# anenbergb/Co-DETR-TensorRT

Measured on AMD Instinct MI355X. Metric: images/sec, Co-DINO Swin-L 1920x1280 fp16 (p50 ms/image alongside), higher is better.
Workload: dtype f16

## Files before the change

### __graft_entry__.py

```python
import os
import subprocess
import sys

ROOT = os.path.dirname(os.path.abspath(__file__))
PKG_ROOT = os.path.join(ROOT, "co-detr-tensorrt_amd")
for _p in (ROOT, PKG_ROOT, os.path.join(ROOT, "oracle")):
    if _p not in sys.path:
        sys.path.insert(0, _p)


def _newer(target, sources):
    if not os.path.isfile(target):
        return True
    t = os.path.getmtime(target)
    return any(os.path.getmtime(s) > t for s in sources)


def build() -> None:
    csrc = os.path.join(PKG_ROOT, "csrc")
    so = os.path.join(PKG_ROOT, "codetr", "libcodetr_hip.so")
    srcs = [os.path.join(csrc, f) for f in os.listdir(csrc) if f.endswith((".hip", ".h", "Makefile"))]
    srcs += [os.path.join(ROOT, "include", h) for h in ("codetr_hip.h", "codetr_jpeg.h", "codetr_assign.h")]
    if _newer(so, srcs):
        subprocess.check_call(["make", "-C", csrc, "-s", "-j4"])
    runner_dir = os.path.join(ROOT, "runner")
    runner = os.path.join(runner_dir, "codetr_runner")
    if _newer(runner, [os.path.join(runner_dir, f) for f in ("codetr_runner.cpp", "dispatch_gen.inc", "Makefile")]):
        subprocess.check_call(["make", "-C", runner_dir, "-s"])
    import msda_oracle

    msda_oracle.build()
    import codetr


def smoke() -> None:
    build()
    import smoke_impl

    smoke_impl.run()


if __name__ == "__main__":
    build()
    print("build ok")
    if len(sys.argv) > 1 and sys.argv[1] == "smoke":
        smoke()
        print("smoke ok")
```

### co-detr-tensorrt_amd/codetr/_kernel_names.py

```python
KERNEL_NAMES = (
    "add_kernel",
    "assign_kernel",
    "batched_nms_kernel",
    "cast_fp8_kernel",
    "cast_fp8mx_kernel",
    "conv_im2col_nchw_kernel",
    "conv_tokens_kernel",
    "decode_boxes_kernel",
    "decoder_layer_kernel",
    "draw_detections_kernel",
    "encoder_geometry_kernel",
    "ffn_fp8_kernel",
    "ffn_fused_kernel",
    "frames_to_rgb_kernel",
    "gather_rows_kernel",
    "gn_apply_kernel",
    "gn_finalize_kernel",
    "gn_partial_kernel",
    "im2col_tokens_kernel",
    "jpeg_encode_rows_kernel",
    "jpeg_gather_rows_kernel",
    "layernorm_fp8_kernel",
    "layernorm_fp8mx_kernel",
    "layernorm_kernel",
    "level_cums_kernel",
    "level_mask_kernel",
    "linear_256_fp8_kernel",
    "linear_256_kernel",
    "linear_kernel",
    "linear_pp_kernel",
    "linear_sk_kernel",
    "linear_xs_kernel",
    "maxpool_tokens_kernel",
    "mha_attention_kernel",
    "msda_backward_generic_kernel",
    "msda_backward_kernel",
    "msda_encoder_v4_kernel",
    "msda_fused_headmajor_kernel",
    "msda_op4_kernel",
    "msda_scalar_kernel",
    "msda_tiled_kernel",
    "pack_w2_kernel",
    "patch_im2col_k4_kernel",
    "postprocess_kernel",
    "postprocess_softnms_kernel",
    "preprocess_batch_kernel",
    "preprocess_kernel",
    "preprocess_tiles_kernel",
    "preprocess_views_kernel",
    "query_sine_embed_kernel",
    "row_max_kernel",
    "sigmoid_kernel",
    "sine_pos_kernel",
    "slice_merge_kernel",
    "splitk_reduce_kernel",
    "swin_mlp_kernel",
    "topk_kernel",
    "topk_reg_kernel",
    "track_update2_kernel",
    "track_update_kernel",
    "tta_merge_kernel",
    "valid_ratios_kernel",
    "window_attention_kernel",
# ... 2 lines not shown
```

### co-detr-tensorrt_amd/codetr/hip_ops.py

```python

import collections
import math

import numpy as np
import torch
import torch.nn.functional as F

from . import _assign, _cabi, _jpeg

NATIVE = {"msda", "linear(f16/bf16, K%64==0)", "layer_norm(f16/bf16)", "swin_window_attention(f16, head_dim 32)",
          "msda_fused(softmax + sampling locations in-kernel)", "groupnorm_tokens(f16, 8 ch/group)",
          "sine_pos_tokens(f16, + level_embed)", "ffn_fused(f16, 256 -> hidden -> 256, ReLU, + identity)",
          "mask_pyramid(level masks + running valid counts + valid ratios)",
          "query_sine_embed(f16: sigmoid x valid ratios + sine embedding of the decoder reference boxes)",
          "encoder_geometry(f16: reference points, proposals, keep/drop state)", "row_max(f16)",
          "preprocess_image(u8 -> f16/f32, cv2-exact resize + pad + normalise + mask)", "batched_nms(f32)",
          "preprocess_batch(u8 -> f16/bf16/f32, <= 32 images of any size per launch, stacked + padded)",
          "postprocess_detections(f16/bf16/f32: threshold + sort + per-class NMS + rescale, one workgroup per image)",
          "postprocess_detections_soft(f16/bf16/f32: threshold + per-class soft-NMS (linear / naive) + max_per_img + rescale)",
          "patch_merge_layernorm(f16: Swin 2x2 gather + LayerNorm)",
          "msda_encoder_packed(f16/bf16: LDS-staged gather for the encoder's self-attention, csrc/msda_encoder4.hip)",
          "patch_embed(f16/bf16: 4x4 patch gather + GEMM)",
          "mha_attention(f16/bf16: dense softmax attention, head_dim 32, <= 1024 keys)",
          "topk(f16/bf16 rows, k <= 1024: radix select + bitonic sort)",
          "im2col_tokens(16-bit token-major maps)",
          "resnet50(f16/bf16: implicit-GEMM conv_tokens, stem window gather + GEMM, maxpool_tokens, BN folded)",
          "small_ops(f16: add, sigmoid, gather_rows, decode_boxes, valid_ratios)",
          "linear_fp8(e4m3 x e4m3, K%128==0) + layer_norm_fp8 + cast_fp8", "ffn_fp8(fused FFN, both products e4m3)"}


LINEAR_PROFILE = None
KERNEL_PROFILE = None


def _timed(name, meta, launch, device):
    if KERNEL_PROFILE is None:
        return launch()
    st = torch.cuda.current_stream(device)
    e0, e1 = torch.cuda.Event(enable_timing=True), torch.cuda.Event(enable_timing=True)
    e0.record(st)
    r = launch()
# ... 69 lines not shown
                    launch = lambda: _cabi.linear_splitk(x2, w, bias, r2, act, out, splits, ws, mk)
                elif (LINEAR_PP and _persistent_ok(mk, head_major, out, x2, w, r2, bias)
                      and _cabi.linear_pp_preferred(x2.shape[0], N, K, act, r2 is not None)):
                    launch = lambda: _cabi.linear_pp(x2, w, bias, r2, act, out)
                elif (_persistent_ok(mk, head_major, out, x2, w, r2, bias)
                      and _cabi.linear_sk_preferred(x2.shape[0], N, K, act, r2 is not None)):
                    launch = lambda: _cabi.linear_sk(x2, w, bias, r2, act, out)
                else:
                    launch = lambda: _cabi.linear(x2, w, bias, r2, act, out, mk, hm_rows, hm_hd)
                _timed_linear(launch, x.device, x2.shape[0], N, K)
        if head_major:
            return out.view(x.shape[0], N // hm_hd, hm_rows, hm_hd)
        return out.view(*x.shape[:-1], N)
    if head_major:
        raise RuntimeError("head_major output exists only on the native linear (f16/bf16, K % 64 == 0)")
    y = F.linear(x, weight, bias)
    if act == "relu_res":
        if row_mask is not None:
            y = y.masked_fill(row_mask[..., None], 0.0)
        return F.relu(y + residual if residual is not None else y)
    if act == "relu":
        y = F.relu(y, inplace=True)
    elif act == "gelu":
        y = F.gelu(y)
    elif act is not None:
        raise ValueError(act)
    if row_mask is not None:
        y = y.masked_fill(row_mask[..., None], 0.0)
    if residual is not None:
        y = y + residual
    return y


LN_GEMM = True


def linear_ln_supported(x, norm_weight, weight):
    return (LN_GEMM and x.is_cuda and norm_weight is not None and norm_weight.dtype == x.dtype and weight.dtype == x.dtype
            and not torch.is_grad_enabled() and norm_weight.shape[0] == x.shape[-1]
            and _cabi.linear_xadd_supported(x.numel() // max(x.shape[-1], 1), weight.shape[0], x.shape[-1], x.dtype))


def linear_ln(x, norm_weight, norm_bias, eps, weight, bias=None, act=None):
    _gpu(x, "linear_ln")
    if linear_ln_supported(x, norm_weight, weight):
        K, N = x.shape[-1], weight.shape[0]
        x2 = x.reshape(-1, K)
        x2 = x2 if x2.is_contiguous() else x2.contiguous()
        w = weight if weight.is_contiguous() else weight.contiguous()
        out = torch.empty((x2.shape[0], N), dtype=x.dtype, device=x.device)
        with torch.cuda.device(x.device):
            ok = _timed_linear(lambda: _cabi.linear_ln(x2, norm_weight, norm_bias, eps, w, bias, act, out),
                               x.device, x2.shape[0], N, K)
        if ok:
            return out.view(*x.shape[:-1], N)
    return linear(layer_norm(x, norm_weight, norm_bias, eps), weight, bias, act=act)


XADD = True
XADD_MIN_ROWS = 0


def linear_xadd_supported(x, x_add, weight):
    return (XADD and x.is_cuda and x_add is not None and x_add.shape == x.shape and x_add.dtype == x.dtype
            and weight.dtype == x.dtype and not torch.is_grad_enabled()
            and x.numel() // max(x.shape[-1], 1) >= XADD_MIN_ROWS
# ... 1472 lines not shown
```

### co-detr-tensorrt_amd/codetr/transformer.py

```python
import math

import torch
import torch.nn as nn

from . import hip_ops
from .multi_scale_deformable_attention import MultiScaleDeformableAttention
from .transformer_layers import BaseTransformerLayer, DetrTransformerDecoderLayer, build_norm


DEC_FUSED = True
DEC_VPROJ = True


class DetrTransformerEncoder(nn.Module):
    def __init__(self, post_norm_cfg=dict(type="LN"), with_cp=-1, transformerlayers=None, num_layers=None,
                 init_cfg=None):
        super().__init__()
        if not isinstance(transformerlayers, dict):
            raise AssertionError("transformerlayers must be a dict")
        layer_cfg = dict(transformerlayers)
        if layer_cfg.pop("type") != "BaseTransformerLayer":
            raise AssertionError("encoder layers must be BaseTransformerLayer")
        self.num_layers = num_layers
        self.layers = nn.ModuleList(BaseTransformerLayer(**layer_cfg) for _ in range(num_layers))
# ... 427 lines not shown
        pos_tokens = [p.flatten(2).transpose(1, 2) for p in mlvl_pos_embeds]
        return self.forward_flat(feat, shapes, mlvl_masks, pos_tokens, reg_branches, cls_branches, forced_topk_indices,
                                 capture)

    def forward_flat(self, feat, shapes, mlvl_masks, mlvl_pos_tokens, reg_branches=None, cls_branches=None,
                     forced_topk_indices=None, capture=None, lvl_pos_embed_flat=None, mask_flat=None,
                     valid_counts=None):
        if not self.as_two_stage:
            raise AssertionError("as_two_stage must be True for DINO")
        dev = feat.device
        mask = mask_flat if mask_flat is not None else torch.cat([m.flatten(1) for m in mlvl_masks], 1)
        if lvl_pos_embed_flat is not None:
            pos = lvl_pos_embed_flat
        else:
            pos = torch.cat([p + self.level_embeds[l].view(1, 1, -1) for l, p in enumerate(mlvl_pos_tokens)], 1)
        spatial_shapes, level_start_index = _shape_tensors(shapes, dev)
        if valid_counts is not None:
            valid_ratios = hip_ops.valid_ratios(valid_counts, _level_wh(shapes, feat.dtype, dev))
        else:
            valid_ratios = torch.stack([get_valid_ratio(m, dtype=feat.dtype) for m in mlvl_masks], 1)
        native_geom = feat.is_cuda and feat.dtype in (torch.float16, torch.bfloat16) and mask.dtype == torch.bool
        if native_geom:
            reference_points, ref_by_level, proposals, row_state = hip_ops.encoder_geometry(valid_ratios, mask, shapes)
            if valid_counts is not None:
                ref_by_level._codetr_valid_counts = valid_counts
        else:
            reference_points = get_reference_points([tuple(s) for s in shapes], valid_ratios, device=dev)
            ref_by_level = reference_points[:, :, None] * valid_ratios[:, None]

        memory = self.encoder.forward_bf(feat, pos, mask, reference_points=ref_by_level, spatial_shapes=spatial_shapes,
                                         level_start_index=level_start_index)
        B = memory.shape[0]
        if native_geom:
            out_mem = hip_ops.linear(memory, self.enc_output.weight, self.enc_output.bias, row_mask=row_state)
        else:
            proposals = make_encoder_output_proposals_export(reference_points, mlvl_masks)
            proposals, out_mem = apply_mask_to_proposal_and_memory(proposals, memory, mask)
            out_mem = hip_ops.linear(out_mem, self.enc_output.weight, self.enc_output.bias)
        out_mem = hip_ops.layer_norm(out_mem, self.enc_output_norm.weight, self.enc_output_norm.bias,
                                     self.enc_output_norm.eps)
        last = self.decoder.num_layers
        cls_head = cls_branches[last]
        enc_cls = hip_ops.linear(out_mem, cls_head.weight, cls_head.bias)
        if forced_topk_indices is None:
            topk = hip_ops.topk(hip_ops.row_max(enc_cls), self.two_stage_num_proposals, want_values=False)[1]
        else:
            topk = forced_topk_indices
        sel = hip_ops.gather_rows(out_mem, topk)
        topk_coords = run_mlp(reg_branches[last], sel, residual=hip_ops.gather_rows(proposals, topk))
        qw = self.query_embed.weight
        if B == 1 or not qw.is_cuda or torch.is_grad_enabled():
            query = qw[None].expand(B, -1, -1)
        else:
            query = hip_ops.derived((qw,), f"_codetr_query_b{B}", lambda: qw.detach()[None].expand(B, -1, -1).contiguous())
        if capture is not None:
            enc_coord = run_mlp(reg_branches[last], out_mem) + proposals
            capture["topk_coords_unact"] = topk_coords
            capture.update(memory=memory, enc_outputs_class=enc_cls, enc_outputs_coord_unact=enc_coord,
                           topk_indices=topk, spatial_shapes=spatial_shapes, level_start_index=level_start_index,
                           valid_ratios=valid_ratios)
        return self.decoder.forward_bf(query, memory, mask, topk_coords, valid_ratios, reg_branches,
                                       spatial_shapes=spatial_shapes, level_start_index=level_start_index)
```

### co-detr-tensorrt_amd/csrc/gemm_f16.hip

```cpp
#include <hip/hip_runtime.h>
#include <type_traits>
#include <stdint.h>
#include <stdlib.h>

#include "codetr_hip.h"
#include "device_prims.h"
#include "gemm_epilogue.h"

namespace {

constexpr int BM = 128, BN = 128;
constexpr int kThreads = 256;
constexpr int kStagingBytes = 4 * 64 * kStagePitch;

template <class F>
__host__ __device__ __forceinline__ auto dispatch_act(int act, F f) {
  switch (act) {
    case 0: return f(std::integral_constant<int, 0>{});
    case 1: return f(std::integral_constant<int, 1>{});
    case 3: return f(std::integral_constant<int, 3>{});
    default: return f(std::integral_constant<int, 2>{});
  }
}

const unsigned short* u16(const void* p) { return static_cast<const unsigned short*>(p); }
struct Operands {
  const unsigned short *x, *w, *b, *r;
  unsigned short* y;
  const unsigned char* mk;
  Operands(const void* X, const void* W, const void* bias, const void* R, void* Y, const void* mask = nullptr)
      : x(u16(X)), w(u16(W)), b(u16(bias)), r(u16(R)), y(static_cast<unsigned short*>(Y)),
        mk(static_cast<const unsigned char*>(mask)) {}
};

template <int BKT>
__device__ __forceinline__ int sw(int row) {
  return BKT == 64 ? (row >> 1) & 7 : ((row >> 2) & 3) ^ (((row >> 2) & 1) << 1);
// ... 51 lines not shown
  static constexpr int P = BKT / 16;
  const unsigned short* src[P];
  int iy[P], ix[P], chunk8[P];
  __device__ __forceinline__ void init(const unsigned short* X, const ConvGeom& g, int M, int m0, int tid) {
    constexpr int CH = BKT / 8;
#pragma unroll
    for (int q = 0; q < P; ++q) {
      const int u = q * kThreads + tid;
      const int r = u / CH, pos = u % CH;
      chunk8[q] = (pos ^ sw<BKT>(r)) * 8;
      int m = m0 + r;
      m = m < M ? m : M - 1;
      const int b = m / g.HoWo, p = m - b * g.HoWo;
      const int oy = p / g.Wo, ox = p - oy * g.Wo;
      src[q] = X + (size_t)b * g.H * g.W * g.C + chunk8[q];
      iy[q] = oy * g.stride - g.pad;
      ix[q] = ox * g.stride - g.pad;
    }
  }
  __device__ __forceinline__ void stage(const ConvGeom& g, int k0, unsigned char* lds_tile, int wave) const {
    const int tap = k0 / g.C, c0 = k0 - tap * g.C;
    const int ky = tap / g.k, kx = tap - ky * g.k;
#pragma unroll
    for (int q = 0; q < P; ++q) {
      const int y = iy[q] + ky, x = ix[q] + kx;
      const unsigned short* s = ((unsigned)y < (unsigned)g.H && (unsigned)x < (unsigned)g.W)
                                    ? src[q] + ((size_t)y * g.W + x) * g.C + c0
                                    : g_conv_zeros + chunk8[q];
      dma_piece(s, lds_tile, q, wave);
    }
  }
};

template <class T, int ACT, bool HAS_BIAS, bool HAS_RES, int BKT, int STAGES, bool SPLITK, bool CONV>
__device__ __forceinline__ void linear_body(const unsigned short* __restrict__ X, const unsigned short* __restrict__ W,
                                            const unsigned short* __restrict__ bias,
                                            const unsigned short* __restrict__ R, unsigned short* __restrict__ Y,
                                            const unsigned char* __restrict__ row_mask, int M, int N, int K,
                                            int tiles_n, int hm_rows, int hm_hd, int kps, const ConvGeom& cg) {
  constexpr int kTileBytes = 128 * BKT * 2;
  constexpr int kStageBytes = 2 * kTileBytes;
  constexpr int LPS = 2 * (BKT / 16);
  constexpr int kLdsBytes = STAGES * kStageBytes > kStagingBytes ? STAGES * kStageBytes : kStagingBytes;
  static_assert(kLdsBytes <= 64 * 1024, "pipeline does not fit 64 KiB");
  static_assert(STAGES >= 2 && STAGES <= 4, "");
  __shared__ __attribute__((aligned(16))) unsigned char lds[kLdsBytes];
  const int tid = threadIdx.x;
  const int lane = tid & 63, wave = tid >> 6;
  const int wm = wave & 1, wn = wave >> 1;

  const unsigned tile = xcd_tile(blockIdx.x, gridDim.x);
  const int tn = tile % tiles_n, tm = tile / tiles_n;
  const int m0 = tm * BM, n0 = tn * BN;

  const int ncol = 4 * (lane >> 4);
  const bool vec_n = (N & 7) == 0;
  f32x4 acc[4][4];
#pragma unroll
  for (int i = 0; i < 4; ++i) {
    f32x4 b4 = {0.f, 0.f, 0.f, 0.f};
    if (HAS_BIAS) {
      const int n = n0 + wn * 64 + i * 16 + ncol;
      if (vec_n) {
        if (n < N) {
          const s16x4 bb = *reinterpret_cast<const s16x4*>(bias + n);
#pragma unroll
          for (int r = 0; r < 4; ++r) b4[r] = T::to_f32((unsigned short)bb[r]);
        }
      } else {
#pragma unroll
        for (int r = 0; r < 4; ++r)
          if (n + r < N) b4[r] = T::to_f32(bias[n + r]);
// ... 66 lines not shown
      const int n = n0 + wn * 64 + i * 16 + ncol;
#pragma unroll
      for (int j = 0; j < 4; ++j) {
        const int m = m0 + wm * 64 + j * 16 + frow;
        if (m >= M || n >= N) continue;
        if (vec_n) {
          *reinterpret_cast<f32x4*>(part + (size_t)m * N + n) = acc[i][j];
        } else {
#pragma unroll
          for (int r = 0; r < 4; ++r)
            if (n + r < N) part[(size_t)m * N + n + r] = acc[i][j][r];
        }
      }
    }
    return;
  }

  if (vec_n) {
    constexpr int kPitch = kStagePitch;
    unsigned char* stage = lds + wave * (64 * kPitch);
#pragma unroll
    for (int i = 0; i < 4; ++i) {
#pragma unroll
      for (int j = 0; j < 4; ++j) {
        float v[4];
#pragma unroll
        for (int r = 0; r < 4; ++r) v[r] = epi_act<ACT, HAS_RES>(acc[i][j][r]);
        *reinterpret_cast<s16x4*>(stage + (j * 16 + frow) * kPitch + (i * 16 + ncol) * 2) = T::pack4(v);
      }
    }
    __builtin_amdgcn_wave_barrier();
    const int srow = lane >> 3, schunk = lane & 7;
    const int n = n0 + wn * 64 + schunk * 8;
    s16x8 rres[8];
    if (HAS_RES) {
#pragma unroll
      for (int it = 0; it < 8; ++it) {
        int m = m0 + wm * 64 + it * 8 + srow;
        m = m < M ? m : M - 1;
        const int nn = n + 8 <= N ? n : (N >= 8 ? N - 8 : 0);
        rres[it] = *reinterpret_cast<const s16x8*>(R + (size_t)m * N + nn);
      }
    }
#pragma unroll
    for (int it = 0; it < 8; ++it) {
      const int ml = it * 8 + srow;
      const int m = m0 + wm * 64 + ml;
      if (m < M && n < N) {
        s16x8 v = *reinterpret_cast<const s16x8*>(stage + ml * kPitch + schunk * 16);
        if (row_mask) {
          const unsigned char mk = row_mask[m];
          if (mk == 2) {
#pragma unroll
            for (int e = 0; e < 8; ++e)
              v[e] = (short)T::from_f32(epi_act<ACT, HAS_RES>(HAS_BIAS ? T::to_f32(bias[n + e]) : 0.f));
          } else if (mk) {
            v = s16x8{0, 0, 0, 0, 0, 0, 0, 0};
          }
        }
        size_t off = (size_t)m * N + n;
        if (hm_hd > 0) off = epi_head_major(m, n, N, hm_rows, hm_hd);
        if (HAS_RES) {
          const s16x8 rr = rres[it];
#pragma unroll
          for (int e = 0; e < 8; ++e) v[e] = (short)epi_residual<T, ACT>((unsigned short)v[e], (unsigned short)rr[e]);
        }
// ... 29 lines not shown
                                                          const unsigned short* __restrict__ W,
                                                          const unsigned short* __restrict__ bias,
                                                          const unsigned short* __restrict__ R,
                                                          unsigned short* __restrict__ Y,
                                                          const unsigned char* __restrict__ row_mask, int M, int N,
                                                          int K, int tiles_n, int hm_rows, int hm_hd, int kps) {
  linear_body<T, ACT, HAS_BIAS, HAS_RES, BKT, STAGES, SPLITK, false>(X, W, bias, R, Y, row_mask, M, N, K, tiles_n,
                                                                     hm_rows, hm_hd, kps, ConvGeom{});
}

template <class T, int ACT, bool HAS_BIAS, bool HAS_RES, int BKT, int STAGES>
__global__ __launch_bounds__(kThreads) void conv_tokens_kernel(const unsigned short* __restrict__ X,
                                                               const unsigned short* __restrict__ W,
                                                               const unsigned short* __restrict__ bias,
                                                               const unsigned short* __restrict__ R,
                                                               unsigned short* __restrict__ Y, int M, int N, int K,
                                                               int tiles_n, ConvGeom cg) {
  linear_body<T, ACT, HAS_BIAS, HAS_RES, BKT, STAGES, false, true>(X, W, bias, R, Y, nullptr, M, N, K, tiles_n, 0, 0, 0,
                                                                   cg);
}

int pipeline_cfg(int64_t K, int64_t tiles) { return (K <= 256 && tiles > 256) ? 322 : 642; }

template <class T, int ACT, int BKT, int STAGES>
int launch_cfg(hipStream_t st, const void* X, const void* W, const void* bias, const void* R, void* Y,
               const void* mask, int M, int N, int K, int hm_rows, int hm_hd) {
  const int tiles_m = (M + BM - 1) / BM, tiles_n = (N + BN - 1) / BN;
  const dim3 grid((unsigned)(tiles_m * tiles_n)), block(kThreads);
  const Operands o(X, W, bias, R, Y, mask);
  if (bias && R) hipLaunchKernelGGL((linear_kernel<T, ACT, true, true, BKT, STAGES, false>), grid, block, 0, st, o.x, o.w, o.b, o.r, o.y, o.mk, M, N, K, tiles_n, hm_rows, hm_hd, 0);
  else if (bias) hipLaunchKernelGGL((linear_kernel<T, ACT, true, false, BKT, STAGES, false>), grid, block, 0, st, o.x, o.w, o.b, o.r, o.y, o.mk, M, N, K, tiles_n, hm_rows, hm_hd, 0);
  else if (R) hipLaunchKernelGGL((linear_kernel<T, ACT, false, true, BKT, STAGES, false>), grid, block, 0, st, o.x, o.w, o.b, o.r, o.y, o.mk, M, N, K, tiles_n, hm_rows, hm_hd, 0);
  else hipLaunchKernelGGL((linear_kernel<T, ACT, false, false, BKT, STAGES, false>), grid, block, 0, st, o.x, o.w, o.b, o.r, o.y, o.mk, M, N, K, tiles_n, hm_rows, hm_hd, 0);
  const hipError_t err = hipGetLastError();
  return err == hipSuccess ? 0 : (int)err;
}

template <class T>
__global__ __launch_bounds__(256) void splitk_reduce_kernel(const float* __restrict__ part,
                                                            const unsigned short* __restrict__ bias,
                                                            const unsigned short* __restrict__ R,
                                                            const unsigned char* __restrict__ row_mask,
                                                            unsigned short* __restrict__ Y, int M, int N, int splits,
                                                            int act) {
  const int ngroups = (N + 3) / 4;
  const long idx = (long)blockIdx.x * 256 + threadIdx.x;
  if (idx >= (long)M * ngroups) return;
  const int m = (int)(idx / ngroups), n = (int)(idx % ngroups) * 4;
  const size_t off = (size_t)m * N + n;
  const bool vec = (N & 3) == 0;
  float v[4] = {0.f, 0.f, 0.f, 0.f};
  for (int z = 0; z < splits; ++z) {
    const float* p = part + (size_t)z * M * N + off;
    if (vec) {
      const f32x4 q = *reinterpret_cast<const f32x4*>(p);
#pragma unroll
      for (int r = 0; r < 4; ++r) v[r] += q[r];
    } else {
#pragma unroll
      for (int r = 0; r < 4; ++r)
        if (n + r < N) v[r] += p[r];
    }
  }
  const unsigned char mk = row_mask ? row_mask[m] : 0;
  dispatch_act(act, [&](auto a) {
#pragma unroll
// ... 27 lines not shown
    return CODETR_E_BADARG;
  if (ws_bytes < (int64_t)splits * M * N * 4) return CODETR_E_BADARG;
  const int ktiles = (int)(K / 64), kps = (ktiles + splits - 1) / splits;
  if ((int64_t)kps * (splits - 1) >= ktiles) return CODETR_E_BADARG;
  const int tiles_m = (int)((M + BM - 1) / BM), tiles_n = (int)((N + BN - 1) / BN);
  const dim3 grid((unsigned)(tiles_m * tiles_n), (unsigned)splits), block(kThreads);
  const Operands o(X, W, bias, R, Y, mask);
  hipLaunchKernelGGL((linear_kernel<T, 0, false, false, 64, 2, true>), grid, block, 0, st, o.x, o.w, nullptr, nullptr,
                     static_cast<unsigned short*>(ws), nullptr, (int)M, (int)N, (int)K, tiles_n, 0, 0, kps);
  const long groups = (long)M * ((N + 3) / 4);
  hipLaunchKernelGGL((splitk_reduce_kernel<T>), dim3((unsigned)((groups + 255) / 256)), dim3(256), 0, st,
                     static_cast<const float*>(ws), o.b, o.r, o.mk, o.y, (int)M, (int)N, splits, act);
  const hipError_t err = hipGetLastError();
  return err == hipSuccess ? 0 : (int)err;
}

template <class T, int ACT>
int launch_act(hipStream_t st, const void* X, const void* W, const void* bias, const void* R, void* Y,
               const void* mask, int M, int N, int K, int hm_rows, int hm_hd) {
  switch (pipeline_cfg(K, (int64_t)((M + BM - 1) / BM) * ((N + BN - 1) / BN))) {
    case 322: return launch_cfg<T, ACT, 32, 2>(st, X, W, bias, R, Y, mask, M, N, K, hm_rows, hm_hd);
    default: return launch_cfg<T, ACT, 64, 2>(st, X, W, bias, R, Y, mask, M, N, K, hm_rows, hm_hd);
  }
}

#ifdef CODETR_GEMM_STAMPS
__device__ unsigned long long* g_stamps = nullptr;
#endif
#ifdef CODETR_GEMM_ABL
constexpr int kGemmAbl = CODETR_GEMM_ABL;
#else
constexpr int kGemmAbl = 0;
#endif
template <class T, int ACT, bool HAS_BIAS, bool HAS_RES, bool XDEEP = false, bool SDMA = false>
__global__ __launch_bounds__(512) void linear_256_kernel(const unsigned short* __restrict__ X,
                                                         const unsigned short* __restrict__ W,
                                                         const unsigned short* __restrict__ bias,
                                                         const unsigned short* __restrict__ R,
                                                         unsigned short* __restrict__ Y,
                                                         const unsigned char* __restrict__ row_mask, int M, int N, int K,
                                                         int tiles_n) {
  constexpr int BKT = 64, NT = 512;
#ifdef CODETR_GEMM_STAMPS
  unsigned long long st0 = 0, st1 = 0, st2 = 0, rt0 = 0;
  if (threadIdx.x == 0) {
    st0 = __builtin_amdgcn_s_memtime();
    rt0 = __builtin_amdgcn_s_memrealtime();
  }
#endif
  constexpr int kTileBytes = 256 * BKT * 2;
  constexpr int kStageBytes = 2 * kTileBytes;
  __shared__ __attribute__((aligned(16))) unsigned char lds[XDEEP ? 5 * kTileBytes : 2 * kStageBytes];
  const int tid = threadIdx.x, lane = tid & 63, wave = tid >> 6;
  const int wm = wave & 1, wn = wave >> 1;
  const unsigned tile = xcd_tile(blockIdx.x, gridDim.x);
  const int tn = tile % tiles_n, tm = tile / tiles_n;
  const int m0 = tm * 256, n0 = tn * 256;
  const int frow = lane & 15, fchunk = lane >> 4, ncol = 4 * (lane >> 4);

  f32x4 acc[4][8];
#pragma unroll
  for (int i = 0; i < 4; ++i) {
    f32x4 b4 = {0.f, 0.f, 0.f, 0.f};
    if (HAS_BIAS) {
      const int n = n0 + wn * 64 + i * 16 + ncol;
      if (n < N) {
        const s16x4 bb = *reinterpret_cast<const s16x4*>(bias + n);
#pragma unroll
        for (int r = 0; r < 4; ++r) b4[r] = T::to_f32((unsigned short)bb[r]);
      }
    }
#pragma unroll
    for (int j = 0; j < 8; ++j) acc[i][j] = b4;
  }
// ... 152 lines not shown
        lds_dma16_auto(gx[q] + koff, nbufX + (q * NT + wave * 64) * 16);
      }
    }
#pragma unroll
    for (int j = 0; j < 8; ++j)
#pragma unroll
      for (int i = 0; i < 4; ++i) {
        if (!(kGemmAbl & 2)) acc[i][j] = T::mfma(a[0][i], b[0][j], acc[i][j]);
        else if (!(kGemmAbl & 4)) asm volatile("" ::"v"(a[0][i]), "v"(b[0][j]));
      }
    __builtin_amdgcn_sched_group_barrier(0x008, 2, 0);
    __builtin_amdgcn_sched_group_barrier(0x100, 12, 0);
#pragma unroll
    for (int g = 0; g < 8; ++g) {
      __builtin_amdgcn_sched_group_barrier(0x008, 3, 0);
      __builtin_amdgcn_sched_group_barrier(0x020, 1, 0);
    }
    __builtin_amdgcn_sched_group_barrier(0x008, 6, 0);
#pragma unroll
    for (int j = 0; j < 8; ++j)
#pragma unroll
      for (int i = 0; i < 4; ++i) {
        if (!(kGemmAbl & 2)) acc[i][j] = T::mfma(a[1][i], b[1][j], acc[i][j]);
        else if (!(kGemmAbl & 4)) asm volatile("" ::"v"(a[1][i]), "v"(b[1][j]));
      }
    __builtin_amdgcn_sched_group_barrier(0x008, 32, 0);
  }
  wait_vmcnt<0>();
  __builtin_amdgcn_s_barrier();
#ifdef CODETR_GEMM_STAMPS
  if (threadIdx.x == 0) st1 = __builtin_amdgcn_s_memtime();
#endif

  constexpr int kPitch = kStagePitch;
  unsigned char* stage = lds + wave * (64 * kPitch);
  const int srow = lane >> 3, schunk = lane & 7;
  const int n = n0 + wn * 64 + schunk * 8;
  unsigned char* ytile = reinterpret_cast<unsigned char*>(Y) + ((size_t)m0 * N + n0) * 2;
#pragma unroll
  for (int h = 0; h < 2; ++h) {
#pragma unroll
    for (int i = 0; i < 4; ++i)
#pragma unroll
      for (int j = 0; j < 4; ++j) {
        float v[4];
#pragma unroll
        for (int r = 0; r < 4; ++r) v[r] = epi_act<ACT, HAS_RES>(acc[i][h * 4 + j][r]);
        *reinterpret_cast<s16x4*>(stage + (j * 16 + frow) * kPitch + (i * 16 + ncol) * 2) = T::pack4(v);
      }
    __builtin_amdgcn_wave_barrier();
    s16x8 rres[8];
    if (HAS_RES) {
#pragma unroll
      for (int it = 0; it < 8; ++it) {
        int m = m0 + wm * 128 + h * 64 + it * 8 + srow;
        m = m < M ? m : M - 1;
        rres[it] = *reinterpret_cast<const s16x8*>(R + (size_t)m * N + epi_residual_col(n, N));
      }
    }
#pragma unroll
    for (int it = 0; it < 8; ++it) {
      const int ml = it * 8 + srow;
      const int m = m0 + wm * 128 + h * 64 + ml;
      if (m < M && n < N) {
        s16x8 v = *reinterpret_cast<const s16x8*>(stage + ml * kPitch + schunk * 16);
        if (row_mask) {
// ... 13 lines not shown
        }
        const unsigned loff = ((unsigned)(wm * 128 + h * 64 + ml) * (unsigned)N + (unsigned)(wn * 64 + schunk * 8)) * 2u;
        *reinterpret_cast<s16x8*>(ytile + loff) = v;
      }
    }
    __builtin_amdgcn_wave_barrier();
  }
#ifdef CODETR_GEMM_STAMPS
  if (threadIdx.x == 0 && g_stamps) {
    st2 = __builtin_amdgcn_s_memtime();
    wait_vmcnt<0>();
    const unsigned long long st3 = __builtin_amdgcn_s_memtime();
    unsigned long long* o = g_stamps + 8 * (size_t)blockIdx.x;
    o[0] = st0; o[1] = st1; o[2] = st2; o[3] = st3; o[4] = rt0; o[5] = __builtin_amdgcn_s_memrealtime();
    o[6] = wait_dma; o[7] = wait_bar;
  }
#endif
}

bool big_applicable(int64_t M, int64_t N, int64_t K, int hm_hd) {
  if (hm_hd != 0 || K < 256 || K % 64 != 0 || N % 8 != 0) return false;
  const int64_t tn = (N + 255) / 256, tm = (M + 255) / 256;
  return tm * tn >= 200 && (N * 8 >= tn * 256 * 7 || (tn == 1 && N * 4 >= 256 * 3));
}

template <class T, int ACT>
int launch_big(hipStream_t st, const void* X, const void* W, const void* bias, const void* R, void* Y, const void* mask,
               int M, int N, int K) {
  const int tiles_m = (M + 255) / 256, tiles_n = (N + 255) / 256;
  const dim3 grid((unsigned)(tiles_m * tiles_n)), block(512);
  const Operands o(X, W, bias, R, Y, mask);
  const bool sdma = tiles_n > 1;
#define CODETR_L256S(HB, HR) \
  hipLaunchKernelGGL((linear_256_kernel<T, ACT, HB, HR, true, true>), grid, block, 0, st, o.x, o.w, o.b, o.r, o.y, o.mk, M, N, K, tiles_n)
#define CODETR_L256(HB, HR) \
  hipLaunchKernelGGL((linear_256_kernel<T, ACT, HB, HR, true, false>), grid, block, 0, st, o.x, o.w, o.b, o.r, o.y, o.mk, M, N, K, tiles_n)
  if (sdma) {
    if (bias && R) CODETR_L256S(true, true);
    else if (bias) CODETR_L256S(true, false);
    else if (R) CODETR_L256S(false, true);
    else CODETR_L256S(false, false);
  } else {
    if (bias && R) CODETR_L256(true, true);
    else if (bias) CODETR_L256(true, false);
    else if (R) CODETR_L256(false, true);
    else CODETR_L256(false, false);
  }
#undef CODETR_L256
#undef CODETR_L256S
  const hipError_t err = hipGetLastError();
  return err == hipSuccess ? 0 : (int)err;
}

#ifndef CODETR_XS_ABL
#define CODETR_XS_ABL 0
#endif
#ifdef CODETR_XS_STAMPS
__device__ unsigned long long* g_xs_stamps = nullptr;
#define XS_STAMP(i) xs_t[i] = __builtin_readcyclecounter()
#else
#define XS_STAMP(i)
#endif
struct XsPosGen {
  const float* ycum[5];
  const float* xcum[5];
  const unsigned short* level_embed;
  int H[5], W[5], start[5];
  int L, S;
  float log2_temperature, scale, eps, offset;
  int normalize;
};

template <class T, int KS, int ACT, bool HAS_RES, class OT = T, bool SPLIT = false, bool POSGEN = false>
__global__ __launch_bounds__(256) void linear_xs_kernel(const unsigned short* __restrict__ X,
                                                        const unsigned short* __restrict__ X2,
                                                        const unsigned short* __restrict__ LNG,
                                                        const unsigned short* __restrict__ LNB, float ln_eps,
                                                        const unsigned short* __restrict__ W,
                                                        const unsigned short* __restrict__ bias,
                                                        const unsigned short* __restrict__ R,
                                                        unsigned short* __restrict__ Y,
                                                        const unsigned char* __restrict__ row_mask, int M, int N, int hm_rows,
// ... 582 lines not shown
                          y_dev, M, N, K, act);
}

int codetr_linear_ln_bf16(void* stream, const void* x_dev, const void* ln_gamma_dev, const void* ln_beta_dev, float ln_eps,
                          const void* w_dev, const void* bias_dev, void* y_dev, int64_t M, int64_t N, int64_t K, int act) {
  return launch_ln<BFloatT>(static_cast<hipStream_t>(stream), x_dev, ln_gamma_dev, ln_beta_dev, ln_eps, w_dev, bias_dev,
                            y_dev, M, N, K, act);
}

int codetr_linear_xadd_f16(void* stream, const void* x_dev, const void* x_add_dev, const void* w_dev,
                           const void* bias_dev, void* y_dev, int64_t M, int64_t N, int64_t K) {
  return launch_xadd<HalfT>(static_cast<hipStream_t>(stream), x_dev, x_add_dev, w_dev, bias_dev, y_dev, M, N, K);
}

int codetr_linear_xadd_bf16(void* stream, const void* x_dev, const void* x_add_dev, const void* w_dev,
                            const void* bias_dev, void* y_dev, int64_t M, int64_t N, int64_t K) {
  return launch_xadd<BFloatT>(static_cast<hipStream_t>(stream), x_dev, x_add_dev, w_dev, bias_dev, y_dev, M, N, K);
}

int codetr_linear_f16(void* stream, const void* x_dev, const void* w_dev, const void* bias_dev, const void* residual_dev,
                      const void* row_mask_dev, void* y_dev, int64_t M, int64_t N, int64_t K, int act, int64_t hm_rows,
                      int hm_head_dim) {
  return launch<HalfT>(static_cast<hipStream_t>(stream), x_dev, w_dev, bias_dev, residual_dev, y_dev, row_mask_dev, M,
                       N, K, act, hm_rows, hm_head_dim);
}

int codetr_linear_bf16(void* stream, const void* x_dev, const void* w_dev, const void* bias_dev,
                       const void* residual_dev, const void* row_mask_dev, void* y_dev, int64_t M, int64_t N,
                       int64_t K, int act, int64_t hm_rows, int hm_head_dim) {
  return launch<BFloatT>(static_cast<hipStream_t>(stream), x_dev, w_dev, bias_dev, residual_dev, y_dev, row_mask_dev,
                         M, N, K, act, hm_rows, hm_head_dim);
}

int codetr_linear_bf16_f16out(void* stream, const void* x_dev, const void* w_dev, const void* bias_dev,
                              const void* row_mask_dev, void* y_dev, int64_t M, int64_t N, int64_t K, int64_t hm_rows,
                              int hm_head_dim) {
  if (!x_dev || !w_dev || !y_dev || M <= 0 || N <= 0 || K <= 0) return CODETR_E_BADARG;
  if (M > 0x7fffffffLL || N > 0x7fffffffLL) return CODETR_E_TOO_LARGE;
  if ((reinterpret_cast<uintptr_t>(x_dev) | reinterpret_cast<uintptr_t>(w_dev) | reinterpret_cast<uintptr_t>(y_dev)) & 15) return CODETR_E_BADARG;
  if (hm_head_dim != 0 || hm_rows != 0) {
    if (hm_head_dim <= 0 || hm_rows <= 0 || hm_head_dim % 8 != 0 || N % hm_head_dim != 0 || M % hm_rows != 0) return CODETR_E_UNSUPPORTED;
  }
  if (!xs_applicable(M, N, K, hm_head_dim) || K == 64) return CODETR_E_UNSUPPORTED;
  hipStream_t st = static_cast<hipStream_t>(stream);
  if (K == 192) return launch_xs_res<BFloatT, 6, 0, HalfT>(st, x_dev, w_dev, bias_dev, nullptr, y_dev, row_mask_dev, (int)M, (int)N, (int)hm_rows, hm_head_dim);
  return launch_xs_res<BFloatT, 8, 0, HalfT>(st, x_dev, w_dev, bias_dev, nullptr, y_dev, row_mask_dev, (int)M, (int)N, (int)hm_rows, hm_head_dim);
}

int codetr_conv_tokens_f16(void* stream, const void* x_dev, const void* w_dev, const void* bias_dev,
                           const void* residual_dev, void* y_dev, int64_t B, int64_t H, int64_t W, int64_t C,
                           int64_t Cout, int k, int stride, int pad, int act) {
  return launch_conv<HalfT>(static_cast<hipStream_t>(stream), x_dev, w_dev, bias_dev, residual_dev, y_dev, B, H, W, C,
                            Cout, k, stride, pad, act);
}

int codetr_conv_tokens_bf16(void* stream, const void* x_dev, const void* w_dev, const void* bias_dev,
                            const void* residual_dev, void* y_dev, int64_t B, int64_t H, int64_t W, int64_t C,
                            int64_t Cout, int k, int stride, int pad, int act) {
  return launch_conv<BFloatT>(static_cast<hipStream_t>(stream), x_dev, w_dev, bias_dev, residual_dev, y_dev, B, H, W, C,
                              Cout, k, stride, pad, act);
}

const char* codetr_linear_variant(int64_t M, int64_t N, int64_t K, int act, int has_residual, int hm_head_dim) {
  if (M <= 0 || N <= 0 || K <= 0 || K % 64 != 0) return "unsupported";
  switch (pick_kernel(M, N, K, act, has_residual != 0, hm_head_dim, true)) {
    case kKernel256: return "tile256";
// ... 27 lines not shown
```

Measured before the change: 99.23.

## Fuse encoder-output LayerNorm into GEMM and class-score row max into linear

Adds a LayerNorm epilogue to the 256-wide GEMM kernel so the encoder output projection and its LayerNorm run in one kernel. It also adds a row-max epilogue to the 128-tile linear kernel so the encoder class head produces per-row maxima directly for top-k, and skips writing the scores unless capture is requested. The aim is to cut two extra kernel launches and the full-size intermediate memory round trips over all encoder tokens. The cost is LDS staging of the whole 256-column tile and an extra barrier, plus new ABI entry points.

```diff
diff --git a/__graft_entry__.py b/__graft_entry__.py
--- a/__graft_entry__.py
+++ b/__graft_entry__.py
@@ -20,7 +20,7 @@
     csrc = os.path.join(PKG_ROOT, "csrc")
     so = os.path.join(PKG_ROOT, "codetr", "libcodetr_hip.so")
     srcs = [os.path.join(csrc, f) for f in os.listdir(csrc) if f.endswith((".hip", ".h", "Makefile"))]
-    srcs += [os.path.join(ROOT, "include", h) for h in ("codetr_hip.h", "codetr_jpeg.h", "codetr_assign.h")]
+    srcs += [os.path.join(ROOT, "include", h) for h in ("codetr_hip.h", "codetr_jpeg.h", "codetr_assign.h", "codetr_head.h")]
     if _newer(so, srcs):
         subprocess.check_call(["make", "-C", csrc, "-s", "-j4"])
     runner_dir = os.path.join(ROOT, "runner")
diff --git a/co-detr-tensorrt_amd/codetr/_head.py b/co-detr-tensorrt_amd/codetr/_head.py
--- /dev/null
+++ b/co-detr-tensorrt_amd/codetr/_head.py
@@ -0,0 +1,66 @@
+import os
+
+from . import _cabi, _cheader
+
+HEADER_PATH = os.path.join(os.path.dirname(_cheader.HEADER_PATH), "codetr_head.h")
+if not os.path.isfile(HEADER_PATH):
+    raise ImportError(f"C ABI header not found at {HEADER_PATH}; the head binding is derived from it")
+with open(HEADER_PATH) as _f:
+    functions, defines = _cheader.parse(_f.read())
+
+ABI_VERSION = defines["CODETR_HEAD_ABI_VERSION"]
+
+SIGNATURES = {name: (_cabi._CTYPE[_cheader.kind(ret, returned=True)], [_cabi._CTYPE[_cheader.kind(t)] for t, _ in params])
+              for name, (ret, params) in functions.items()}
+
+_lib = None
+
+
+def load():
+    global _lib
+    if _lib is not None:
+        return _lib
+    _cabi.load()
+    lib = _cabi._lib
+    for name, (res, args) in SIGNATURES.items():
+        try:
+            fn = getattr(lib, name)
+        except AttributeError as e:
+            raise ImportError(f"{_cabi.LIB_PATH} does not export {name}; rebuild the extension") from e
+        fn.restype = res
+        fn.argtypes = args
+    ver = lib.codetr_head_abi_version()
+    if ver != ABI_VERSION:
+        raise ImportError(f"{_cabi.LIB_PATH} has head ABI version {ver}, host expects {ABI_VERSION}; rebuild the extension")
+    _lib = lib
+    return lib
+
+
+def recording() -> bool:
+    return _cabi.RECORDER is not None
+
+
+def linear_layernorm(x2d, weight, bias, row_mask, ln_weight, ln_bias, eps, out2d):
+    _cabi.CALLS["linear"] += 1
+    _cabi.CALLS["linear_tile256"] += 1
+    M, K = x2d.shape
+    name = "codetr_linear_layernorm_" + _cabi._SUFFIX[x2d.dtype]
+    rc = getattr(load(), name)(
+        _cabi.current_stream_ptr(x2d.device), x2d.data_ptr(), weight.data_ptr(),
+        bias.data_ptr() if bias is not None else None, row_mask.data_ptr() if row_mask is not None else None,
+        ln_weight.data_ptr(), ln_bias.data_ptr(), float(eps), out2d.data_ptr(), M, weight.shape[0], K)
+    _cabi.check(rc, name)
+    return out2d
+
+
+def linear_rowmax(x2d, weight, bias, out2d, row_max):
+    _cabi.CALLS["linear"] += 1
+    _cabi.CALLS["linear_tile128"] += 1
+    M, K = x2d.shape
+    name = "codetr_linear_rowmax_" + _cabi._SUFFIX[x2d.dtype]
+    rc = getattr(load(), name)(
+        _cabi.current_stream_ptr(x2d.device), x2d.data_ptr(), weight.data_ptr(),
+        bias.data_ptr() if bias is not None else None, out2d.data_ptr() if out2d is not None else None,
+        row_max.data_ptr(), M, weight.shape[0], K)
+    _cabi.check(rc, name)
+    return row_max
diff --git a/co-detr-tensorrt_amd/codetr/_kernel_names.py b/co-detr-tensorrt_amd/codetr/_kernel_names.py
--- a/co-detr-tensorrt_amd/codetr/_kernel_names.py
+++ b/co-detr-tensorrt_amd/codetr/_kernel_names.py
@@ -29,6 +29,7 @@
     "linear_256_kernel",
     "linear_kernel",
     "linear_pp_kernel",
+    "linear_rowmax_kernel",
     "linear_sk_kernel",
     "linear_xs_kernel",
     "maxpool_tokens_kernel",
diff --git a/co-detr-tensorrt_amd/codetr/hip_ops.py b/co-detr-tensorrt_amd/codetr/hip_ops.py
--- a/co-detr-tensorrt_amd/codetr/hip_ops.py
+++ b/co-detr-tensorrt_amd/codetr/hip_ops.py
@@ -6,7 +6,7 @@
 import torch
 import torch.nn.functional as F
 
-from . import _assign, _cabi, _jpeg
+from . import _assign, _cabi, _head, _jpeg
 
 NATIVE = {"msda", "linear(f16/bf16, K%64==0)", "layer_norm(f16/bf16)", "swin_window_attention(f16, head_dim 32)",
           "msda_fused(softmax + sampling locations in-kernel)", "groupnorm_tokens(f16, 8 ch/group)",
@@ -142,6 +142,61 @@
     return y
 
 
+LINEAR_LN_OUT = True
+
+
+def linear_layernorm(x, weight, bias, ln_weight, ln_bias, eps, row_mask=None):
+    _gpu(x, "linear_layernorm")
+    K, N = x.shape[-1], weight.shape[0]
+    M = x.numel() // K if K else 0
+    fused = (LINEAR_LN_OUT and not _head.recording() and N == 256 and M > 0 and _cabi.linear_supported(x, weight)
+             and ln_weight is not None and ln_bias is not None and ln_weight.dtype == ln_bias.dtype == x.dtype
+             and _cabi.linear_variant(M, N, K) == "tile256")
+    if fused:
+        x2 = x.reshape(-1, K)
+        if not x2.is_contiguous():
+            x2 = x2.contiguous()
+        w = weight if weight.is_contiguous() else weight.contiguous()
+        mk = None
+        if row_mask is not None:
+            mk = row_mask.reshape(-1)
+            if mk.dtype != torch.bool and mk.dtype != torch.uint8:
+                mk = mk != 0
+            mk = mk.contiguous()
+        out = torch.empty((M, N), dtype=x.dtype, device=x.device)
+        operands = (x2, w, bias, ln_weight, ln_bias, out)
+        persistent = mk is None and ((LINEAR_PP and _cabi.linear_pp_preferred(M, N, K)) or _cabi.linear_sk_preferred(M, N, K))
+        if not persistent and all(t is None or (t.is_contiguous() and t.data_ptr() % 16 == 0) for t in operands):
+            with torch.cuda.device(x.device):
+                _timed_linear(lambda: _head.linear_layernorm(x2, w, bias, mk, ln_weight, ln_bias, eps, out), x.device, M, N, K)
+            return out.view(*x.shape[:-1], N)
+    return layer_norm(linear(x, weight, bias, row_mask=row_mask), ln_weight, ln_bias, eps)
+
+
+LINEAR_ROWMAX = True
+
+
+def linear_row_max(x, weight, bias=None, want_scores=True):
+    _gpu(x, "linear_row_max")
+    K, N = x.shape[-1], weight.shape[0]
+    M = x.numel() // K if K else 0
+    if (LINEAR_ROWMAX and not _head.recording() and M > 0 and N % 8 == 0 and N <= 128 and _cabi.linear_supported(x, weight)
+            and _cabi.linear_variant(M, N, K) == "tile128" and _cabi.linear_splitk_plan(M, N, K)[0] == 1
+            and not (LINEAR_PP and _cabi.linear_pp_preferred(M, N, K)) and not _cabi.linear_sk_preferred(M, N, K)):
+        x2 = x.reshape(-1, K)
+        if not x2.is_contiguous():
+            x2 = x2.contiguous()
+        w = weight if weight.is_contiguous() else weight.contiguous()
+        if x2.data_ptr() % 16 == 0 and w.data_ptr() % 16 == 0 and (bias is None or bias.data_ptr() % 16 == 0):
+            out = torch.empty((M, N), dtype=x.dtype, device=x.device) if want_scores else None
+            mx = torch.empty((M,), dtype=x.dtype, device=x.device)
+            with torch.cuda.device(x.device):
+                _timed_linear(lambda: _head.linear_rowmax(x2, w, bias, out, mx), x.device, M, N, K)
+            return (out.view(*x.shape[:-1], N) if want_scores else None), mx.view(x.shape[:-1])
+    y = linear(x, weight, bias)
+    return (y if want_scores else None), row_max(y)
+
+
 LN_GEMM = True
 
 
diff --git a/co-detr-tensorrt_amd/codetr/transformer.py b/co-detr-tensorrt_amd/codetr/transformer.py
--- a/co-detr-tensorrt_amd/codetr/transformer.py
+++ b/co-detr-tensorrt_amd/codetr/transformer.py
@@ -483,19 +483,23 @@
                                          level_start_index=level_start_index)
         B = memory.shape[0]
         if native_geom:
-            out_mem = hip_ops.linear(memory, self.enc_output.weight, self.enc_output.bias, row_mask=row_state)
+            out_mem = hip_ops.linear_layernorm(memory, self.enc_output.weight, self.enc_output.bias,
+                                               self.enc_output_norm.weight, self.enc_output_norm.bias,
+                                               self.enc_output_norm.eps, row_mask=row_state)
         else:
             proposals = make_encoder_output_proposals_export(reference_points, mlvl_masks)
             proposals, out_mem = apply_mask_to_proposal_and_memory(proposals, memory, mask)
             out_mem = hip_ops.linear(out_mem, self.enc_output.weight, self.enc_output.bias)
-        out_mem = hip_ops.layer_norm(out_mem, self.enc_output_norm.weight, self.enc_output_norm.bias,
-                                     self.enc_output_norm.eps)
+            out_mem = hip_ops.layer_norm(out_mem, self.enc_output_norm.weight, self.enc_output_norm.bias,
+                                         self.enc_output_norm.eps)
         last = self.decoder.num_layers
         cls_head = cls_branches[last]
-        enc_cls = hip_ops.linear(out_mem, cls_head.weight, cls_head.bias)
         if forced_topk_indices is None:
-            topk = hip_ops.topk(hip_ops.row_max(enc_cls), self.two_stage_num_proposals, want_values=False)[1]
-        else:
+            enc_cls, enc_max = hip_ops.linear_row_max(out_mem, cls_head.weight, cls_head.bias,
+                                                      want_scores=capture is not None)
+            topk = hip_ops.topk(enc_max, self.two_stage_num_proposals, want_values=False)[1]
+        else:
+            enc_cls = hip_ops.linear(out_mem, cls_head.weight, cls_head.bias)
             topk = forced_topk_indices
         sel = hip_ops.gather_rows(out_mem, topk)
         topk_coords = run_mlp(reg_branches[last], sel, residual=hip_ops.gather_rows(proposals, topk))
diff --git a/co-detr-tensorrt_amd/csrc/gemm_f16.hip b/co-detr-tensorrt_amd/csrc/gemm_f16.hip
--- a/co-detr-tensorrt_amd/csrc/gemm_f16.hip
+++ b/co-detr-tensorrt_amd/csrc/gemm_f16.hip
@@ -3,6 +3,7 @@
 #include <stdint.h>
 #include <stdlib.h>
 
+#include "codetr_head.h"
 #include "codetr_hip.h"
 #include "device_prims.h"
 #include "gemm_epilogue.h"
@@ -120,12 +121,14 @@
   }
 };
 
-template <class T, int ACT, bool HAS_BIAS, bool HAS_RES, int BKT, int STAGES, bool SPLITK, bool CONV>
+template <class T, int ACT, bool HAS_BIAS, bool HAS_RES, int BKT, int STAGES, bool SPLITK, bool CONV, bool ROWMAX = false>
 __device__ __forceinline__ void linear_body(const unsigned short* __restrict__ X, const unsigned short* __restrict__ W,
                                             const unsigned short* __restrict__ bias,
                                             const unsigned short* __restrict__ R, unsigned short* __restrict__ Y,
                                             const unsigned char* __restrict__ row_mask, int M, int N, int K,
-                                            int tiles_n, int hm_rows, int hm_hd, int kps, const ConvGeom& cg) {
+                                            int tiles_n, int hm_rows, int hm_hd, int kps, const ConvGeom& cg,
+                                            unsigned short* __restrict__ row_max_out = nullptr) {
+  static_assert(!ROWMAX || (!HAS_RES && !SPLITK && !CONV), "the row maximum: a plain linear's rows");
   constexpr int kTileBytes = 128 * BKT * 2;
   constexpr int kStageBytes = 2 * kTileBytes;
   constexpr int LPS = 2 * (BKT / 16);
@@ -258,6 +261,50 @@
     __builtin_amdgcn_wave_barrier();
     const int srow = lane >> 3, schunk = lane & 7;
     const int n = n0 + wn * 64 + schunk * 8;
+    if (ROWMAX) {
+      float rm[8];
+#pragma unroll
+      for (int it = 0; it < 8; ++it) {
+        const int ml = it * 8 + srow;
+        const int m = m0 + wm * 64 + ml;
+        float mx = -__builtin_inff();
+        int nan = 0;
+        if (m < M && n < N) {
+          s16x8 v = *reinterpret_cast<const s16x8*>(stage + ml * kPitch + schunk * 16);
+          if (row_mask) epi_row_state<T, T, ACT, HAS_RES>(v, row_mask[m], HAS_BIAS, bias, n);
+#pragma unroll
+          for (int e = 0; e < 8; ++e) {
+            const float f = T::to_f32((unsigned short)v[e]);
+            nan |= f != f;
+            mx = f > mx ? f : mx;
+          }
+          if (Y) *reinterpret_cast<s16x8*>(Y + (size_t)m * N + n) = v;
+        }
+#pragma unroll
+        for (int o = 4; o > 0; o >>= 1) {
+          const float m2 = __shfl_xor(mx, o, 64);
+          nan |= __shfl_xor(nan, o, 64);
+          mx = m2 > mx ? m2 : mx;
+        }
+        rm[it] = nan ? __builtin_nanf("") : mx;
+      }
+      __builtin_amdgcn_wave_barrier();
+      if (wn == 1 && schunk == 0) {
+#pragma unroll
+        for (int it = 0; it < 8; ++it) reinterpret_cast<float*>(stage)[it * 8 + srow] = rm[it];
+      }
+      __syncthreads();
+      if (wn == 0 && schunk == 0) {
+        const float* other = reinterpret_cast<const float*>(lds + (wave + 2) * (64 * kPitch));
+#pragma unroll
+        for (int it = 0; it < 8; ++it) {
+          const int m = m0 + wm * 64 + it * 8 + srow;
+          const float a = rm[it], b = other[it * 8 + srow];
+          if (m < M) row_max_out[m] = T::from_f32((a != a || b != b) ? __builtin_nanf("") : (b > a ? b : a));
+        }
+      }
+      return;
+    }
     s16x8 rres[8];
     if (HAS_RES) {
 #pragma unroll
@@ -353,6 +400,42 @@
   else if (bias) hipLaunchKernelGGL((linear_kernel<T, ACT, true, false, BKT, STAGES, false>), grid, block, 0, st, o.x, o.w, o.b, o.r, o.y, o.mk, M, N, K, tiles_n, hm_rows, hm_hd, 0);
   else if (R) hipLaunchKernelGGL((linear_kernel<T, ACT, false, true, BKT, STAGES, false>), grid, block, 0, st, o.x, o.w, o.b, o.r, o.y, o.mk, M, N, K, tiles_n, hm_rows, hm_hd, 0);
   else hipLaunchKernelGGL((linear_kernel<T, ACT, false, false, BKT, STAGES, false>), grid, block, 0, st, o.x, o.w, o.b, o.r, o.y, o.mk, M, N, K, tiles_n, hm_rows, hm_hd, 0);
+  const hipError_t err = hipGetLastError();
+  return err == hipSuccess ? 0 : (int)err;
+}
+
+template <class T, bool HAS_BIAS, int BKT, int STAGES>
+__global__ __launch_bounds__(kThreads) void linear_rowmax_kernel(const unsigned short* __restrict__ X,
+                                                                 const unsigned short* __restrict__ W,
+                                                                 const unsigned short* __restrict__ bias,
+                                                                 unsigned short* __restrict__ Y,
+                                                                 unsigned short* __restrict__ row_max_out, int M, int N,
+                                                                 int K) {
+  linear_body<T, 0, HAS_BIAS, false, BKT, STAGES, false, false, true>(X, W, bias, nullptr, Y, nullptr, M, N, K, 1, 0, 0, 0,
+                                                                      ConvGeom{}, row_max_out);
+}
+
+template <class T>
+int launch_rowmax(hipStream_t st, const void* X, const void* W, const void* bias, void* Y, void* rowmax, int64_t M,
+                  int64_t N, int64_t K) {
+  if (!X || !W || !rowmax || M <= 0 || N <= 0 || K <= 0) return CODETR_E_BADARG;
+  if (K % 64 != 0 || N % 8 != 0 || N > BN) return CODETR_E_UNSUPPORTED;
+  if (M > 0x7fffffffLL - BM || K > 0x7fffffffLL) return CODETR_E_TOO_LARGE;
+  if ((reinterpret_cast<uintptr_t>(X) | reinterpret_cast<uintptr_t>(W) | reinterpret_cast<uintptr_t>(Y)) & 15)
+    return CODETR_E_BADARG;
+  if ((reinterpret_cast<uintptr_t>(bias) & 7) || (reinterpret_cast<uintptr_t>(rowmax) & 1)) return CODETR_E_BADARG;
+  const int tiles_m = (int)((M + BM - 1) / BM);
+  const dim3 grid((unsigned)tiles_m), block(kThreads);
+  const Operands o(X, W, bias, nullptr, Y);
+  unsigned short* rm = static_cast<unsigned short*>(rowmax);
+  const bool shallow = pipeline_cfg(K, tiles_m) == 322;
+#define CODETR_ROWMAX(HB, BKT) \
+  hipLaunchKernelGGL((linear_rowmax_kernel<T, HB, BKT, 2>), grid, block, 0, st, o.x, o.w, o.b, o.y, rm, (int)M, (int)N, (int)K)
+  if (bias && shallow) CODETR_ROWMAX(true, 32);
+  else if (bias) CODETR_ROWMAX(true, 64);
+  else if (shallow) CODETR_ROWMAX(false, 32);
+  else CODETR_ROWMAX(false, 64);
+#undef CODETR_ROWMAX
   const hipError_t err = hipGetLastError();
   return err == hipSuccess ? 0 : (int)err;
 }
@@ -446,14 +529,43 @@
 #else
 constexpr int kGemmAbl = 0;
 #endif
-template <class T, int ACT, bool HAS_BIAS, bool HAS_RES, bool XDEEP = false, bool SDMA = false>
+template <class T>
+__device__ __forceinline__ s16x8 ln_row8(s16x8 v, s16x8 gw, s16x8 gb, float eps) {
+  const float inv_c = 1.0f / 256.f;
+  auto group_sum = [](float x) {
+#pragma unroll
+    for (int o = 16; o > 0; o >>= 1) x += __shfl_xor(x, o, 64);
+    return x;
+  };
+  float s = 0.f;
+#pragma unroll
+  for (int e = 0; e < 8; ++e) s += T::to_f32((unsigned short)v[e]);
+  const float mean = group_sum(s) * inv_c;
+  float q = 0.f;
+#pragma unroll
+  for (int e = 0; e < 8; ++e) {
+    const float d = T::to_f32((unsigned short)v[e]) - mean;
+    q = fmaf(d, d, q);
+  }
+  const float rstd = rsqrtf(group_sum(q) * inv_c + eps);
+  s16x8 o;
+#pragma unroll
+  for (int e = 0; e < 8; ++e)
+    o[e] = (short)T::from_f32(fmaf((T::to_f32((unsigned short)v[e]) - mean) * rstd, T::to_f32((unsigned short)gw[e]),
+                                   T::to_f32((unsigned short)gb[e])));
+  return o;
+}
+
+template <class T, int ACT, bool HAS_BIAS, bool HAS_RES, bool XDEEP = false, bool SDMA = false, bool LN = false>
 __global__ __launch_bounds__(512) void linear_256_kernel(const unsigned short* __restrict__ X,
                                                          const unsigned short* __restrict__ W,
                                                          const unsigned short* __restrict__ bias,
                                                          const unsigned short* __restrict__ R,
                                                          unsigned short* __restrict__ Y,
                                                          const unsigned char* __restrict__ row_mask, int M, int N, int K,
-                                                         int tiles_n) {
+                                                         int tiles_n, const unsigned short* __restrict__ ln_gamma,
+                                                         const unsigned short* __restrict__ ln_beta, float ln_eps) {
+  static_assert(!LN || (XDEEP && !HAS_RES && ACT == 0), "the LayerNorm epilogue: whole-tile staging, plain rows");
   constexpr int BKT = 64, NT = 512;
 #ifdef CODETR_GEMM_STAMPS
   unsigned long long st0 = 0, st1 = 0, st2 = 0, rt0 = 0;
@@ -672,6 +784,40 @@
   if (threadIdx.x == 0) st1 = __builtin_amdgcn_s_memtime();
 #endif
 
+  if (LN) {
+    constexpr int kLnPitch = 256 * 2 + 32;
+    static_assert(!LN || 256 * kLnPitch <= (int)sizeof(lds), "");
+    const int sub = tid & 31, rloc = tid >> 5;
+    const s16x8 gw = *reinterpret_cast<const s16x8*>(ln_gamma + sub * 8);
+    const s16x8 gb = *reinterpret_cast<const s16x8*>(ln_beta + sub * 8);
+    unsigned char mk[16];
+#pragma unroll
+    for (int it = 0; it < 16; ++it) {
+      const int m = m0 + it * 16 + rloc;
+      mk[it] = row_mask ? row_mask[m < M ? m : M - 1] : (unsigned char)0;
+    }
+#pragma unroll
+    for (int j = 0; j < 8; ++j)
+#pragma unroll
+      for (int i = 0; i < 4; ++i) {
+        float v[4];
+#pragma unroll
+        for (int r = 0; r < 4; ++r) v[r] = epi_act<ACT, HAS_RES>(acc[i][j][r]);
+        *reinterpret_cast<s16x4*>(lds + (wm * 128 + j * 16 + frow) * kLnPitch + (wn * 64 + i * 16 + ncol) * 2) = T::pack4(v);
+      }
+    __syncthreads();
+    unsigned char* yt = reinterpret_cast<unsigned char*>(Y) + (size_t)m0 * 256 * 2;
+#pragma unroll
+    for (int it = 0; it < 16; ++it) {
+      const int ml = it * 16 + rloc;
+      s16x8 v = *reinterpret_cast<const s16x8*>(lds + ml * kLnPitch + sub * 16);
+      epi_row_state<T, T, ACT, HAS_RES>(v, mk[it], HAS_BIAS, bias, sub * 8);
+      const s16x8 o = ln_row8<T>(v, gw, gb, ln_eps);
+      if (m0 + ml < M) *reinterpret_cast<s16x8*>(yt + ((unsigned)ml * 256u + (unsigned)sub * 8u) * 2u) = o;
+    }
+    return;
+  }
+
   constexpr int kPitch = kStagePitch;
   unsigned char* stage = lds + wave * (64 * kPitch);
   const int srow = lane >> 3, schunk = lane & 7;
@@ -751,9 +897,9 @@
   const Operands o(X, W, bias, R, Y, mask);
   const bool sdma = tiles_n > 1;
 #define CODETR_L256S(HB, HR) \
-  hipLaunchKernelGGL((linear_256_kernel<T, ACT, HB, HR, true, true>), grid, block, 0, st, o.x, o.w, o.b, o.r, o.y, o.mk, M, N, K, tiles_n)
+  hipLaunchKernelGGL((linear_256_kernel<T, ACT, HB, HR, true, true>), grid, block, 0, st, o.x, o.w, o.b, o.r, o.y, o.mk, M, N, K, tiles_n, nullptr, nullptr, 0.f)
 #define CODETR_L256(HB, HR) \
-  hipLaunchKernelGGL((linear_256_kernel<T, ACT, HB, HR, true, false>), grid, block, 0, st, o.x, o.w, o.b, o.r, o.y, o.mk, M, N, K, tiles_n)
+  hipLaunchKernelGGL((linear_256_kernel<T, ACT, HB, HR, true, false>), grid, block, 0, st, o.x, o.w, o.b, o.r, o.y, o.mk, M, N, K, tiles_n, nullptr, nullptr, 0.f)
   if (sdma) {
     if (bias && R) CODETR_L256S(true, true);
     else if (bias) CODETR_L256S(true, false);
@@ -767,6 +913,27 @@
   }
 #undef CODETR_L256
 #undef CODETR_L256S
+  const hipError_t err = hipGetLastError();
+  return err == hipSuccess ? 0 : (int)err;
+}
+
+template <class T>
+int launch_big_ln(hipStream_t st, const void* X, const void* W, const void* bias, const void* mask, const void* G,
+                  const void* Bt, float eps, void* Y, int64_t M, int64_t N, int64_t K) {
+  if (!X || !W || !G || !Bt || !Y || M <= 0 || N <= 0 || K <= 0) return CODETR_E_BADARG;
+  if (N != 256 || K % 64 != 0) return CODETR_E_UNSUPPORTED;
+  if (M > 0x7fffffffLL - 256 || K > 0x7fffffffLL) return CODETR_E_TOO_LARGE;
+  if ((reinterpret_cast<uintptr_t>(X) | reinterpret_cast<uintptr_t>(W) | reinterpret_cast<uintptr_t>(bias) |
+       reinterpret_cast<uintptr_t>(G) | reinterpret_cast<uintptr_t>(Bt) | reinterpret_cast<uintptr_t>(Y)) & 15)
+    return CODETR_E_BADARG;
+  const dim3 grid((unsigned)((M + 255) / 256)), block(512);
+  const Operands o(X, W, bias, nullptr, Y, mask);
+  if (bias)
+    hipLaunchKernelGGL((linear_256_kernel<T, 0, true, false, true, false, true>), grid, block, 0, st, o.x, o.w, o.b, o.r, o.y,
+                       o.mk, (int)M, 256, (int)K, 1, u16(G), u16(Bt), eps);
+  else
+    hipLaunchKernelGGL((linear_256_kernel<T, 0, false, false, true, false, true>), grid, block, 0, st, o.x, o.w, o.b, o.r, o.y,
+                       o.mk, (int)M, 256, (int)K, 1, u16(G), u16(Bt), eps);
   const hipError_t err = hipGetLastError();
   return err == hipSuccess ? 0 : (int)err;
 }
@@ -1415,6 +1582,32 @@
                          M, N, K, act, hm_rows, hm_head_dim);
 }
 
+int codetr_head_abi_version(void) { return CODETR_HEAD_ABI_VERSION; }
+
+int codetr_linear_layernorm_f16(void* stream, const void* x_dev, const void* w_dev, const void* bias_dev,
+                                const void* row_mask_dev, const void* ln_gamma_dev, const void* ln_beta_dev, float ln_eps,
+                                void* y_dev, int64_t M, int64_t N, int64_t K) {
+  return launch_big_ln<HalfT>(static_cast<hipStream_t>(stream), x_dev, w_dev, bias_dev, row_mask_dev, ln_gamma_dev,
+                              ln_beta_dev, ln_eps, y_dev, M, N, K);
+}
+
+int codetr_linear_layernorm_bf16(void* stream, const void* x_dev, const void* w_dev, const void* bias_dev,
+                                 const void* row_mask_dev, const void* ln_gamma_dev, const void* ln_beta_dev, float ln_eps,
+                                 void* y_dev, int64_t M, int64_t N, int64_t K) {
+  return launch_big_ln<BFloatT>(static_cast<hipStream_t>(stream), x_dev, w_dev, bias_dev, row_mask_dev, ln_gamma_dev,
+                                ln_beta_dev, ln_eps, y_dev, M, N, K);
+}
+
+int codetr_linear_rowmax_f16(void* stream, const void* x_dev, const void* w_dev, const void* bias_dev, void* y_dev,
+                             void* row_max_dev, int64_t M, int64_t N, int64_t K) {
+  return launch_rowmax<HalfT>(static_cast<hipStream_t>(stream), x_dev, w_dev, bias_dev, y_dev, row_max_dev, M, N, K);
+}
+
+int codetr_linear_rowmax_bf16(void* stream, const void* x_dev, const void* w_dev, const void* bias_dev, void* y_dev,
+                              void* row_max_dev, int64_t M, int64_t N, int64_t K) {
+  return launch_rowmax<BFloatT>(static_cast<hipStream_t>(stream), x_dev, w_dev, bias_dev, y_dev, row_max_dev, M, N, K);
+}
+
 int codetr_linear_bf16_f16out(void* stream, const void* x_dev, const void* w_dev, const void* bias_dev,
                               const void* row_mask_dev, void* y_dev, int64_t M, int64_t N, int64_t K, int64_t hm_rows,
                               int hm_head_dim) {
diff --git a/include/codetr_head.h b/include/codetr_head.h
--- /dev/null
+++ b/include/codetr_head.h
@@ -0,0 +1,29 @@
+#ifndef CODETR_HEAD_H_
+#define CODETR_HEAD_H_
+
+#include <stdint.h>
+
+#include "codetr_hip.h"
+
+#ifdef __cplusplus
+extern "C" {
+#endif
+
+#define CODETR_HEAD_ABI_VERSION 1
+
+int codetr_head_abi_version(void);
+int codetr_linear_layernorm_f16(void *stream, const void *x_dev, const void *w_dev, const void *bias_dev,
+                                const void *row_mask_dev, const void *ln_gamma_dev, const void *ln_beta_dev,
+                                float ln_eps, void *y_dev, int64_t M, int64_t N, int64_t K);
+int codetr_linear_layernorm_bf16(void *stream, const void *x_dev, const void *w_dev, const void *bias_dev,
+                                 const void *row_mask_dev, const void *ln_gamma_dev, const void *ln_beta_dev,
+                                 float ln_eps, void *y_dev, int64_t M, int64_t N, int64_t K);
+int codetr_linear_rowmax_f16(void *stream, const void *x_dev, const void *w_dev, const void *bias_dev, void *y_dev,
+                             void *row_max_dev, int64_t M, int64_t N, int64_t K);
+int codetr_linear_rowmax_bf16(void *stream, const void *x_dev, const void *w_dev, const void *bias_dev, void *y_dev,
+                              void *row_max_dev, int64_t M, int64_t N, int64_t K);
+
+#ifdef __cplusplus
+}
+#endif
+#endif
```

Measured after the change: 99.61, median of 6. About the same (+0.4%).
